# wildminder/ComfyUI-KEEP

Measured on AMD Instinct MI355X. Metric: restored 512x512 face frames/sec, T=20 clip, higher is better.
Workload: dtype f16x3; 1 GPU; 48 independent clips x T=20 x 512x512 per GPU (BASELINE configs[1] clips), KEEP config, synthetic weights seed 0, precision policy x3; clips_per_gpu=48, clip_length=20, parallelism=dp1 over clips, precision_policy=x3

## Files before the change

comfyui-keep_amd/csrc/keep_attn.hip:

```cpp
#include <math.h>
#include <stdlib.h>

#include <type_traits>

#include "keep_common.h"

static constexpr int KEEP_NT_ATTN_O = 0;


struct AttnP {
  const float* q;
  const float* k;
  const float* v;
  const unsigned short* q16;
  const unsigned short* k16;
  const unsigned short* v16;
  float* o;
  long q_bs, q_ts, q_hs, k_bs, k_ts, k_hs, v_bs, v_ts, v_hs, o_bs, o_ts, o_hs;
  int B, H, Lq, Lk, D, Dv;
  float scale;
  int mode, T, seg_len;
  int img_h, img_w, ksplit, shift, kv_rot, n_img;
  int nslices;
  unsigned flags;
  const _Float16* kv_pack;
  const float* q_amax;
  const float* k_amax;
  const float* v_amax;
};

enum AttnForm {
  ATTN_F32,
  ATTN_BF16,
  ATTN_BF16IN,
  ATTN_X3_NQ8,
  ATTN_X3_NQ16,
  ATTN_X3_NQ0,
  ATTN_X3_PACKED,
  ATTN_X3_SMALL,
  ATTN_X3_TWO_PASS,
  ATTN_X3_SFULL,
  ATTN_X3_SFULL2,
};
struct AttnPlan {
  AttnForm form;
  int waves;
  int dvt;
  bool masked;
  size_t lds;
  int64_t scratch;
};
// ... 878 lines not shown
        pl[j] = (_Float16)(s[st * 8 + j] - (float)h);
      }
#pragma unroll
      for (int j = 0; j < DVT; ++j) {
        const _Float16* vrow = Vt + (j * 32 + l31) * VP + (st * 2 + lhi) * 8;
        const af16x8 vh8 = *reinterpret_cast<const af16x8*>(vrow), vl8 = *reinterpret_cast<const af16x8*>(vrow + 32);
        o[j] = __builtin_amdgcn_mfma_f32_32x32x16_f16(pl, vh8, o[j], 0, 0, 0);
        o[j] = __builtin_amdgcn_mfma_f32_32x32x16_f16(ph, vl8, o[j], 0, 0, 0);
        o[j] = __builtin_amdgcn_mfma_f32_32x32x16_f16(ph, vh8, o[j], 0, 0, 0);
      }
    }
    if (PF && kt + 1 < ntiles) {
      __syncthreads();
      if (PACKED) {
        pk_commit();
      } else {
        k_commit();
        v_commit();
      }
    }
  }

  const float inv_l = inv_sv / l_run;
#pragma unroll
  for (int r = 0; r < 16; ++r) {
    const int qrow = (r & 3) + 8 * (r >> 2) + 4 * lhi;
    const float il = __shfl(inv_l, qrow);
    const int t = q0 + wave * 32 + qrow;
    if (t < p.Lq) {
      const long base = q_offset(p, b, t, p.o_bs, p.o_ts) + (long)head * p.o_hs;
#pragma unroll
      for (int j = 0; j < DVT; ++j) {
        const int dv = dv0 + j * 32 + l31;
        if (dv >= p.Dv) continue;
        if (KEEP_NT_ATTN_O)
          __builtin_nontemporal_store(o[j][r] * il, p.o + base + dv);
        else
          p.o[base + dv] = o[j][r] * il;
      }
    }
  }
}

template <int DC, int DVS>
__global__ __launch_bounds__(256) void attn_pack_kv_x3_kernel(AttnP p, _Float16* out) {
  constexpr int QP = 2 * DC + 8, VP = 72, PKK = 32 * QP / 8, PKV = DVS * VP / 8;
// ... 1149 lines not shown
    KEEP_REQUIRE(a.ksplit > 0 && a.img_h % a.ksplit == 0 && a.img_w % a.ksplit == 0, "keep_attention: bad window split");
    const int wh = a.img_h / a.ksplit, ww = a.img_w / a.ksplit;
    KEEP_REQUIRE(a.Lq == wh * ww && a.Lk == wh * ww, "keep_attention: window mode needs Lq == Lk == window size");
    KEEP_REQUIRE(a.n_img > 0 && a.B == a.n_img * a.ksplit * a.ksplit, "keep_attention: B != n_img*ksplit^2");
    KEEP_REQUIRE(a.shift == 0 || a.shift == wh / 2, "keep_attention: shift=%d must be 0 or img_h/ksplit/2 = %d", a.shift, wh / 2);
    KEEP_REQUIRE(a.kv_rot >= 0 && a.kv_rot < a.n_img, "keep_attention: bad kv_rot");
    KEEP_REQUIRE((long)a.img_h * a.img_w <= 65536, "keep_attention: window mode supports maps of at most 65536 tokens");
  }
  KEEP_REQUIRE((!a.q_amax && !a.k_amax && !a.v_amax) || (a.q_amax && a.k_amax && a.v_amax && a.mode == 0 && a.mma == KEEP_MMA_X3),
               "keep_attention: q/k/v_amax come together, with KEEP_MMA_X3 and mode 0 only");
  p.flags = a.flags;
  p.q = (const float*)a.q; p.k = (const float*)a.k; p.v = (const float*)a.v; p.o = a.o;
  p.q16 = (const unsigned short*)a.q; p.k16 = (const unsigned short*)a.k; p.v16 = (const unsigned short*)a.v;
  p.q_bs = a.q_bs; p.q_ts = a.q_ts; p.q_hs = a.q_hs;
  p.k_bs = a.k_bs; p.k_ts = a.k_ts; p.k_hs = a.k_hs;
  p.v_bs = a.v_bs; p.v_ts = a.v_ts; p.v_hs = a.v_hs;
  p.o_bs = a.o_bs; p.o_ts = a.o_ts; p.o_hs = a.o_hs;
  p.B = a.B; p.H = a.H; p.Lq = a.Lq; p.Lk = a.Lk; p.D = a.D; p.Dv = a.Dv;
  p.scale = a.scale; p.mode = a.mode; p.T = a.T; p.seg_len = a.seg_len;
  p.img_h = a.img_h; p.img_w = a.img_w; p.ksplit = a.ksplit; p.shift = a.shift; p.kv_rot = a.kv_rot;
  p.n_img = a.n_img;
  p.q_amax = a.q_amax; p.k_amax = a.k_amax; p.v_amax = a.v_amax;
  p.kv_pack = nullptr;
  const int dvt = a.Dv <= 32 ? 1 : (a.Dv <= 64 ? 2 : 4);
  p.nslices = cdiv(a.Dv, dvt * 32);
  pl = AttnPlan{ATTN_F32, a.Lq <= 32 ? 1 : 4, dvt, false, 0, 0};

  auto rows16 = [](const void* base, int64_t bs, int64_t ts, int64_t hs, int n) {
    return bs % n == 0 && ts % n == 0 && hs % n == 0 && (uintptr_t)base % 16 == 0;
  };
  const int DC = a.D < 128 ? a.D : 128;
  const size_t ntl = (size_t)(a.Lk + 31) / 32;
  const size_t win_tables = ntl * 32 * 4 + ntl * 16 + ntl * 32;

  if (a.in_dtype == KEEP_BF16) {
    const bool ok = a.mma == KEEP_MMA_BF16 && a.D % 16 == 0 && a.Dv % 8 == 0 && rows16(a.q, a.q_bs, a.q_ts, a.q_hs, 8) &&
                    rows16(a.k, a.k_bs, a.k_ts, a.k_hs, 8) && rows16(a.v, a.v_bs, a.v_ts, a.v_hs, 8);
    KEEP_REQUIRE(ok, "keep_attention: bf16 inputs need KEEP_MMA_BF16, D %% 16 == 0, Dv %% 8 == 0 and 16-byte aligned rows");
    const size_t operands = (size_t)((128 + 64) * (DC + 8) + dvt * 32 * 72) * 2;
    const size_t staging = (size_t)4 * 32 * (dvt * 32 + 4) * 4;
    pl.form = ATTN_BF16IN;
    pl.waves = 4;
    pl.masked = a.mode == 2 && a.shift > 0;
    pl.lds = (128 + 3 * 64 + 3 * 64) * sizeof(long) + 3 * 16 * sizeof(unsigned long long) + (operands > staging ? operands : staging);
    return KEEP_OK;
  }
  const bool qk16 = a.D % 16 == 0 && rows16(a.q, a.q_bs, a.q_ts, a.q_hs, 4) && rows16(a.k, a.k_bs, a.k_ts, a.k_hs, 4);
  if (a.mma == KEEP_MMA_BF16) {
    KEEP_REQUIRE(qk16, "keep_attention: KEEP_MMA_BF16 needs D %% 16 == 0 and 16-byte aligned q/k rows");
    pl.form = ATTN_BF16;
    pl.lds = (size_t)((pl.waves * 32 + 32) * (DC + 8) + dvt * 32 * 40) * 2;
    return KEEP_OK;
  }
  if (a.mma != KEEP_MMA_X3 || !qk16 || (a.flags & KEEP_ATTN_NO_X3)) {
    pl.lds = (size_t)((pl.waves * 32 + 32) * (DC + 1) + 32 * dvt * 32) * sizeof(float);
    return KEEP_OK;
  }
// ... 49 lines not shown

template <class F>
static int with_dvt(int dvt, F f) {
  if (dvt == 1) return f(std::integral_constant<int, 1>{});
  if (dvt == 2) return f(std::integral_constant<int, 2>{});
  return f(std::integral_constant<int, 4>{});
}

extern "C" int32_t keep_sizeof_attention_args(void) { return (int32_t)sizeof(keep_attention_args); }

extern "C" int64_t keep_attention_workspace_bytes(const keep_attention_args* a_in) {
  keep_attention_args a;
  AttnP p;
  AttnPlan pl;
  if (attn_args_in(a_in, a) != KEEP_OK || plan_attention(a, INT64_MAX, p, pl) != KEEP_OK) return 0;
  return pl.scratch;
}

extern "C" int32_t keep_attention(const keep_attention_args* a_in, void* stream) {
  keep_attention_args a;
  const int rc_in = attn_args_in(a_in, a);
  if (rc_in != KEEP_OK) return rc_in;
  KEEP_REQUIRE(a.q && a.k && a.v && a.o, "keep_attention: null tensor pointer");
  AttnP p;
  AttnPlan pl;
  const bool ws_ok = a.workspace && (uintptr_t)a.workspace % 16 == 0;
  const int rc = plan_attention(a, ws_ok ? a.workspace_bytes : 0, p, pl);
  if (rc != KEEP_OK) return rc;
  hipStream_t st = (hipStream_t)stream;
  const bool one_wave = pl.waves == 1;
  switch (pl.form) {
    case ATTN_F32:
      return with_dvt(pl.dvt, [&](auto dvt) {
        return one_wave ? launch_attn<1, decltype(dvt)::value>(p, pl, st) : launch_attn<4, decltype(dvt)::value>(p, pl, st);
      });
    case ATTN_BF16:
      return with_dvt(pl.dvt, [&](auto dvt) {
        return one_wave ? launch_attn_bf16<1, decltype(dvt)::value>(p, pl, st) : launch_attn_bf16<4, decltype(dvt)::value>(p, pl, st);
      });
    case ATTN_BF16IN:
      return with_dvt(pl.dvt, [&](auto dvt) { return launch_attn_bf16in<decltype(dvt)::value>(p, pl, st); });
    case ATTN_X3_NQ8:
      return with_dvt(pl.dvt, [&](auto dvt) {
        return one_wave ? launch_attn_x3_t<1, decltype(dvt)::value, 8>(p, pl, st) : launch_attn_x3_t<4, decltype(dvt)::value, 8>(p, pl, st);
      });
    case ATTN_X3_NQ16:
// ... 300 lines not shown
```

comfyui-keep_amd/engine/hiplib.py:

```python
import ctypes as C
import os

import torch

_HERE = os.path.dirname(os.path.abspath(__file__))
LIB_PATH = os.environ.get('KEEP_HIP_LIB') or os.path.join(os.path.dirname(_HERE), 'csrc', 'libkeep_hip.so')
ABI_VERSION = 23

F32, BF16 = 0, 1
MMA_F32, MMA_BF16, MMA_X3, MMA_X1 = 0, 1, 2, 3
PRO_NONE, PRO_SWISH, PRO_RELU = 0, 1, 2
ACT_NONE, ACT_RELU, ACT_LRELU02, ACT_GELU, ACT_SIGMOID, ACT_LRELU01, ACT_SILU = 0, 1, 2, 3, 4, 5, 6
PAD_ZERO, PAD_REFLECT = 0, 1
UPSAMPLE_X2_PHASES = 2
(CONV_NO_COUT4, CONV_NO_C3, CONV_NO_HALO_F32, CONV_NO_HALO_X3, CONV_NO_GATHER_X3, CONV_NO_PLAIN, CONV_NO_FLATK_F32,
 CONV_SMALL_TILES, CONV_X3_EXACT_ACT, CONV_NO_STREAM, CONV_NO_GEMM_LAT, CONV_GEMM_LAT_WAVES, CONV_GEMM_LAT_TILES, CONV_NO_SMALL_PARTIALS) = (1 << i for i in range(14))
CONV_X1_HALO16 = 1 << 15
CONV_X1_GEMM = 1 << 14
ATTN_NO_PACK, ATTN_NO_SFULL2, ATTN_NO_X3, ATTN_NO_SMALL, ATTN_NO_TWO_PASS = 1, 2, 4, 8, 16

_vp, _i32, _i64, _f32, _u32 = C.c_void_p, C.c_int32, C.c_int64, C.c_float, C.c_uint32
STATUS_NONFINITE_LOGITS, STATUS_NONFINITE_TENSOR = 1, 2


class ConvArgs(C.Structure):
    _fields_ = [('struct_size', _u32), ('flags', _u32), ('inp', _vp), ('weight', _vp), ('bias', _vp), ('out', _vp), ('pro_scale', _vp), ('pro_shift', _vp),
                ('residual', _vp), ('aux', _vp), ('workspace', _vp)] + \
               [(n, _i32) for n in ('N', 'H', 'W', 'Cin', 'Cout', 'KH', 'KW', 'stride', 'pad_t', 'pad_l', 'Ho', 'Wo',
                                    'in_ld', 'out_ld', 'res_ld', 'upsample', 'pro_act', 'epi_act')] + \
               [('aux_w', _f32), ('split_k', _i32), ('dtype', _i32), ('mma', _i32), ('weight_bf16', _vp), ('stats_out', _vp), ('stats_P', _i32), ('bk256', _i32), ('out_dtype', _i32),
                ('weight_x3', _vp), ('x3_acc_scale', _f32), ('x3_in_amax', _vp), ('x3_out_amax', _vp), ('x3_out_amax_zeroed', _i32), ('in2', _vp), ('in2_cin1', _i32), ('pad_mode', _i32),
                ('ln_gamma', _vp), ('ln_beta', _vp), ('ln_eps', _f32), ('plan_ref_images', _i32)]


class ConvPlanOut(C.Structure):
    _fields_ = [('path', _i32), ('split_k', _i32), ('workspace_bytes', _i64), ('stats_rows', _i32), ('stats_P', _i32),
                ('wants_bf16_input', _i32), ('out_bf16_ok', _i32), ('out_amax_ok', _i32), ('kernel', C.c_char * 64)]


class AttnArgs(C.Structure):
    _fields_ = [('struct_size', _u32), ('flags', _u32), ('q', _vp), ('k', _vp), ('v', _vp), ('o', _vp)] + \
               [(n, _i64) for n in ('q_bs', 'q_ts', 'q_hs', 'k_bs', 'k_ts', 'k_hs', 'v_bs', 'v_ts', 'v_hs',
                                    'o_bs', 'o_ts', 'o_hs')] + \
               [(n, _i32) for n in ('B', 'H', 'Lq', 'Lk', 'D', 'Dv')] + [('scale', _f32), ('mode', _i32)] + \
               [(n, _i32) for n in ('T', 'seg_len', 'img_h', 'img_w', 'ksplit', 'shift', 'kv_rot', 'n_img', 'mma', 'in_dtype')] + \
               [('q_amax', _vp), ('k_amax', _vp), ('v_amax', _vp), ('workspace', _vp), ('workspace_bytes', _i64)]


_SIGNATURES = {
    'keep_conv2d': [C.POINTER(ConvArgs), _vp],
    'keep_conv2d_plan': [C.POINTER(ConvArgs), C.POINTER(ConvPlanOut)],
    'keep_attention': [C.POINTER(AttnArgs), _vp],
    'keep_chan_stats': [_vp, _vp, _i32, _i32, _i32, _i32, _i32, _vp],
    'keep_norm_finalize': [_vp, _vp, _vp, _vp, _vp, _i32, _i32, _i32, _i32, _i32, _f32, _vp],
    'keep_group_stats': [_vp, _vp, _vp, _vp, _vp, _i32, _i32, _i32, _i32, _f32, _vp],
    'keep_affine_act': [_vp, _vp, _vp, _vp, _i32, _i32, _i32, _i32, _vp],
    'keep_gm_mlp': [_vp, _vp, _vp, _vp, _vp, _i64, _i32, _vp],
    'keep_token_linear': [_vp, _vp, _vp, _vp, _i64, _i32, _i32, _i32, _vp],
    'keep_gm_ffn_x3': [_vp, _vp, _vp, _f32, _vp, _f32, _vp, _vp, _f32, _vp, _i64, _i32, _i32, _i32, _vp],
    'keep_norm_act_bf16': [_vp, _vp, _vp, _vp, _i32, _i32, _i32, _i32, _i32, _vp],
    'keep_gm_join': [_vp, _vp, _vp, _vp, _vp, _vp, _vp, _i32, _i32, _i32, _vp],
    'keep_bilinear_upscale': [_vp, _vp, _i32, _i32, _i32, _i32, _vp],
    'keep_absmax': [_vp, _vp, _i32, _i64, _i32, _i64, _i64, _i32, _vp],
    'keep_layernorm': [_vp, _vp, _vp, _vp, _vp, _vp, _i32, _vp, _i32, _i32, _f32, _vp],
    'keep_geglu': [_vp, _vp, _i32, _i32, _vp],
    'keep_layernorm_amax': [_vp, _vp, _vp, _vp, _vp, _i32, _i32, _f32, _i32, _vp, _i32, _vp],
    'keep_geglu_amax': [_vp, _vp, _i32, _i32, _i32, _vp, _i32, _vp],
    'keep_argmax_gather': [_vp, _vp, _vp, _vp, _vp, _vp, _i32, _i32, _i32, _vp, _vp],
    'keep_nonfinite_flag': [_vp, _i64, _vp, _vp],
# ... 147 lines not shown
```

comfyui-keep_amd/engine/net.py:

```python
import math
import os

import numpy as np
import torch

from . import hiplib as L
from . import ops
from .arch import (CHANNELS, DEFAULT_ARCH, FUSE_ENCODER_BLOCK, FUSE_GENERATOR_BLOCK, GMFLOW, encoder_blocks,
                   generator_blocks)
from .weights import logical_tensors, pack_blob, validate_state_dict, views

_KNOWN_KW = set(DEFAULT_ARCH) | {
    'gumbel_straight_through', 'gumbel_kl_weight', 'vqgan_path', 'fix_modules', 'flownet_path', 'cfa_nlayers',
    'cross_residual', 'mask_ratio'}


FUSED_GM_MLP = os.environ.get('KEEP_NO_FUSED_MLP') is None
FUSED_GM_FFN_X3 = os.environ.get('KEEP_X3_FUSED_FFN', '1') != '0'
GM_S2D_CONV1 = os.environ.get('KEEP_GM_S2D', '1') != '0'
GM_DEDUP_L0 = os.environ.get('KEEP_GM_DEDUP_L0', '1') != '0'
CHECK_X3_RANGE = os.environ.get('KEEP_X3_NO_RANGE_CHECK') is None
GRAPH_MAX_CLIPS = int(os.environ.get('KEEP_AMD_GRAPH_MAX_CLIPS', '2'))
STREAM_OVERLAP_MAX_CLIPS = int(os.environ.get('KEEP_AMD_OVERLAP_MAX_CLIPS', '2'))
CFT_SPLIT = os.environ.get('KEEP_CFT_SPLIT', '1') != '0'
# ... 125 lines not shown
                 and not n.startswith('flownet.')]
        self._dev_blobx1, self._x1_ranges = ops.make_x1_blob(self._dev_blob, self._index, self.w, names)
        x3 = {(a, b): s for a, b, s in self._x3_scales}
        assert all(x3.get((a, b)) == s for a, b, s in self._x1_ranges), 'x1 and x3 twins must share their per-tensor scales'

    def twin_bytes(self, precision=None):
        precision = self.precision if precision is None else precision
        n = int(self._dev_blob.numel()) if self._dev_blob is not None else (0 if self._blob is None else int(self._blob.size))
        return {'bf16': 2 * n, 'x3': 4 * n, 'f16': 4 * n + 2 * n}.get(precision, 0)

    def _activate_precision(self):
        if self.precision == 'bf16':
            if self._dev_blob16 is None:
                self._dev_blob16 = self._dev_blob.to(torch.bfloat16)
            self.o.set_precision(L.MMA_BF16, self._dev_blob, self._dev_blob16)
        elif self.precision in ('x3', 'f16'):
            if self._dev_blobx3 is None:
                self._make_x3()
            self.o.set_precision(L.MMA_X3, self._dev_blob, None, self._dev_blobx3, 1.0, x3_scales=self._x3_scales)
            if FUSED_GM_FFN_X3:
                for n_ in self.w:
                    if n_.startswith('flownet.') and n_.endswith('.mlp.2.weight') and self.w[n_].shape[0] == 128:
                        self.o.ffn_w2_twin(self.w[n_])
            if ops.UP2_PHASES:
                for i, (kind, _, _) in enumerate(generator_blocks(self.cfg)):
                    if kind == 'up':
                        self.o.up2_twin(self.w[f'generator.blocks.{i}.conv.weight'])
            if self.precision == 'f16':
                if self._dev_blobx1 is None:
                    self._make_x1()
                self.o.set_x1_twin(self._dev_blobx1, self._x1_ranges, flags=0, base_kernel=ops.X3_STREAM_KERNEL)
        else:
            self.o.set_precision(L.MMA_F32, self._dev_blob, None)

    def _upload(self, from_blob=None):
        L.load(check_device=True)
        if from_blob is None:
            if self._pinned is None:
                self._pinned = torch.from_numpy(self._blob).pin_memory()
            from_blob = self._pinned
        self._dev_blob = from_blob.to(self.device, non_blocking=False)
        self._dev_blob16 = self._dev_blobx3 = self._dev_blobx1 = None
        self._graphs = {}
        self.w = views(self._dev_blob, self._index)

    def to(self, device):
# ... 282 lines not shown

    def _gm_resblock(self, x, p, stride):
        w = self.w
        c1, st1 = self.o.conv(x, w[f'{p}.conv1.weight'], None, stride=stride, pad=1, stats=True, bounded=True)
        c2, st2 = self.o.conv(c1, w[f'{p}.conv2.weight'], None, pro=self._inorm(c1, st1), pro_act=L.PRO_RELU, stats=True)
        s2, h2 = self._inorm(c2, st2)
        N, H, Wd, C = c2.shape
        out = torch.empty_like(c2)
        if f'{p}.downsample.0.weight' in w:
            d, std = self.o.conv(x, w[f'{p}.downsample.0.weight'].view(C, 1, 1, -1), w[f'{p}.downsample.0.bias'],
                                 stride=stride, pad=0, ksize=1, stats=True, bounded=True)
            sd, hd = self._inorm(d, std)
            L.call('keep_gm_join', d, sd, hd, c2, s2, h2, out, N, H * Wd, C)
        else:
            L.call('keep_gm_join', x, None, None, c2, s2, h2, out, N, H * Wd, C)
        return out

    def _gm_layer(self, src, tgt, p, ffn, h8, w8, shift, kv_rot, n_img):
        w = self.w
        C = src.shape[-1]
        Ltok = h8 * w8
        wqkv = w[f'{p}.qkv.weight']
        o = torch.empty_like(src)
        if tgt is src:
            qkv = self.o.linear(src, wqkv, out_bf16=True, bounded=True, n_img=n_img)
            q, k, v = qkv, ops.offset(qkv, C), ops.offset(qkv, 2 * C)
            sq = skv = (Ltok * 3 * C, 3 * C, 0)
        else:
            q = self.o.linear(src, wqkv[:C], out_bf16=True, bounded=True, n_img=n_img)
            kv = self.o.linear(tgt, wqkv[C:], out_bf16=True, bounded=True, n_img=n_img)
            k, v = kv, ops.offset(kv, C)
            sq, skv = (Ltok * C, C, 0), (Ltok * 2 * C, 2 * C, 0)
        self.o.attention(q, k, v, o, B=n_img * 4, H=1, Lq=Ltok // 4, Lk=Ltok // 4, D=C, Dv=C, scale=1.0 / (C ** 0.5),
                      q_str=sq, k_str=skv, v_str=skv, o_str=(Ltok * C, C, 0), mode=2, img_h=h8, img_w=w8, ksplit=2,
                      shift=shift, kv_rot=kv_rot, n_img=n_img)
        n1 = (w[f'{p}.norm1.weight'], w[f'{p}.norm1.bias'], 1e-5)
        fuse = self.o.ln_fusable(w[f'{p}.merge.weight'], Ltok)
        if not ffn:
            if fuse:
                return self.o.linear(o, w[f'{p}.merge.weight'], bounded=True, n_img=n_img, ln=n1, residual=src)
            m = self.o.linear(o, w[f'{p}.merge.weight'], bounded=True, n_img=n_img)
            return ops.layernorm(m, n1[0], n1[1], res=src)
        if fuse:
            m = self.o.linear(o, w[f'{p}.merge.weight'], bounded=True, n_img=n_img, ln=n1)
        else:
            m = ops.layernorm(self.o.linear(o, w[f'{p}.merge.weight'], bounded=True, n_img=n_img), n1[0], n1[1])
        if (self.o.mma == L.MMA_X3 and C == 128 and FUSED_GM_FFN_X3 and self.o.x3_twin(w[f'{p}.mlp.0.weight']) is not None):
            return self.o.gm_ffn_x3(src, m, w[f'{p}.mlp.0.weight'], w[f'{p}.mlp.2.weight'], w[f'{p}.norm2.weight'], w[f'{p}.norm2.bias'], 1e-5)
        if self.o.mma == L.MMA_BF16 and C == 128 and FUSED_GM_MLP:
            m2 = self.o.gm_mlp(src, m, w[f'{p}.mlp.0.weight'], w[f'{p}.mlp.2.weight'])
        else:
            if self.o.mma == L.MMA_X3:
                hmid = self.o.linear(src, w[f'{p}.mlp.0.weight'], act=L.ACT_GELU, bounded=True, x2=m, n_img=n_img)
            else:
                hmid = self.o.linear(ops.concat2(src, m), w[f'{p}.mlp.0.weight'], act=L.ACT_GELU, bounded=True, n_img=n_img)
            if self.o.ln_fusable(w[f'{p}.mlp.2.weight'], Ltok):
                return self.o.linear(hmid, w[f'{p}.mlp.2.weight'], bounded=True, n_img=n_img, residual=src,
                                     ln=(w[f'{p}.norm2.weight'], w[f'{p}.norm2.bias'], 1e-5))
            m2 = self.o.linear(hmid, w[f'{p}.mlp.2.weight'], bounded=True, n_img=n_img)
        return ops.layernorm(m2, w[f'{p}.norm2.weight'], w[f'{p}.norm2.bias'], res=src)

    def _gm_backbone(self, img_nchw):
        w = self.w
        pfx = 'flownet.model'
        ws2d = w.get(f'{pfx}.backbone.conv1.weight_s2d') if GM_S2D_CONV1 else None
        if ws2d is not None and img_nchw.shape[2] % 2 == 0 and img_nchw.shape[3] % 2 == 0:
# ... 441 lines not shown
```

comfyui-keep_amd/engine/ops.py:

```python
import bisect
import os

import torch

from . import hiplib as L

TOKEN_LINEAR = os.environ.get('KEEP_NO_TOKEN_LINEAR') is None
UP2_PHASES = os.environ.get('KEEP_X3_UP2', '1') != '0'
FUSE_LN = os.environ.get('KEEP_X3_FUSE_LN', '1') != '0'
USE_BK256 = bool(int(os.environ.get('KEEP_BK256', '0')))
HALO_PRENORM_MINPIX = int(os.environ.get('KEEP_HALO_PRENORM_MINPIX', '0'))

DEBUG_SYNC = os.environ.get('KEEP_DEBUG_SYNC') is not None
X3_STREAM_KERNEL = 'conv3x3_halo_x3s_kernel'
_PLAN_CACHE = {}
POLICY_NAMES = {L.MMA_F32: 'fp32', L.MMA_BF16: 'bf16', L.MMA_X3: 'x3'}
PLAN_REF_IMAGES = int(os.environ.get('KEEP_PLAN_REF_IMAGES', '0') or 0)
DEFAULT_CONV_FLAGS = L.CONV_X3_EXACT_ACT if os.environ.get('KEEP_X3_EXACT_ACT') else 0


class Plan:
    __slots__ = ('split_k', 'ws_floats', 'stats_P', 'wants_bf16_input', 'out_bf16_ok', 'out_amax_ok', 'kernel')

    def __init__(self, o):
        self.split_k = o.split_k
        self.ws_floats = o.workspace_bytes // 4
        self.stats_P = o.stats_P
        self.wants_bf16_input = bool(o.wants_bf16_input)
        self.out_bf16_ok = bool(o.out_bf16_ok)
        self.out_amax_ok = bool(o.out_amax_ok)
        self.kernel = o.kernel.decode()
# ... 31 lines not shown
    def __init__(self):
        self.mma = L.MMA_F32
        self.attn_mma = L.MMA_F32
        self.blob32 = None
        self.blob16 = None
        self.blobx3 = None
        self.x3_acc_scale = 1.0
        self._x3_table = None
        self._up2, self._up2_src = {}, (None, None)
        self.profile = None
        self.amax_arena = None
        self.amax_pos = 0
        self.status = None
        self.arena_generation = 0
        self.flags = DEFAULT_CONV_FLAGS
        self.attn_flags = 0
        self.plan_ref_images = PLAN_REF_IMAGES
        self.blobx1 = None
        self._x1_table = None
        self._x1_route = {}
        self.x1_flags = L.CONV_X1_GEMM
        self.x1_base = L.MMA_X3
        self.x1_base_kernel = None
        self.census = None

    def begin_forward(self, device):
        self.ensure_arena(device)
        self._block.zero_()
        self.amax_pos = 0

    def ensure_arena(self, device):
        device = torch.device(device)
        if self.amax_arena is None or self.amax_arena.device != device:
            self._block = torch.empty((1 << 18) + 4, dtype=torch.float32, device=device)
            self.amax_arena = self._block[4:]
            self.status = self._block[:1].view(torch.int32)
            self.arena_generation += 1

    def set_precision(self, mma, blob32=None, blob16=None, blobx3=None, x3_acc_scale=1.0, x3_scales=None):
        if mma not in (L.MMA_F32, L.MMA_BF16, L.MMA_X3):
            raise ValueError(f"set_precision: {mma!r} is no base policy (single fp16 is a base policy plus set_x1_twin)")
        self._x3_table = ([a for a, _, _ in x3_scales], list(x3_scales)) if x3_scales else None
        self.mma = self.attn_mma = mma
        self.set_x1_twin()
        if blobx3 is not None and (blob32 is not self._up2_src[0] or blobx3 is not self._up2_src[1]):
            self._up2, self._up2_src = {}, (blob32, blobx3)
# ... 43 lines not shown

    def bf16_twin(self, w):
        if self.blob16 is None:
            raise RuntimeError("bf16 policy needs the bf16 blob registered (Ops.set_precision)")
        off = self._blob_off(w)
        return self.blob16[off:off + w.numel()]

    def up2_twin(self, w):
        key = (w.data_ptr(), tuple(w.shape))
        tw = self._up2.get(key)
        if tw is None:
            w4 = up2_phase_weights(w)
            sc = x3_scale_for(float(w4.abs().max()))
            tw = self._up2[key] = (split_x3(w4.reshape(-1, w.shape[-1]), sc).view(-1), 1.0 / sc)
        return tw

    def ffn_w2_twin(self, w2):
        key = ('ffn_w2', w2.data_ptr(), tuple(w2.shape))
        tw = self._up2.get(key)
        if tw is None:
            wp = ffn_w2_perm(w2)
            sc = x3_scale_for(float(wp.abs().max()))
            tw = self._up2[key] = (split_x3(wp, sc).view(-1), 1.0 / sc)
        return tw

    def gm_ffn_x3(self, src, msg, w0, w2, gamma, beta, eps):
        C = src.shape[-1]
        M = src.numel() // C
        out = empty((M, C), src)
        w2p, asc2 = self.ffn_w2_twin(w2)
        if self.profile is not None:
            e0, e1 = torch.cuda.Event(enable_timing=True), torch.cuda.Event(enable_timing=True)
            Hd = w0.shape[0]
            self.profile.append(('gm_ffn_x3_kernel', 2.0 * M * (2 * C * Hd + Hd * C), 1, e0, e1,
                                 3 * M * C * 4 + (2 * C * Hd + Hd * C) * 4, (M // 4096 if M % 4096 == 0 else 1, M, 1, 2 * C, C, 1, 1, 0, False)))
            e0.record()
        L.call('keep_gm_ffn_x3', src, msg, self.x3_twin(w0), float(self.x3_scale_of(w0)), w2p, float(asc2), gamma, beta, float(eps), out,
               M, C, w0.shape[0], 1 if (self.flags & L.CONV_X3_EXACT_ACT) else 0)
        if self.profile is not None:
            self.profile[-1][4].record()
        return out.view(src.shape)

    def x3_twin(self, w):
        if self.blobx3 is None or w.shape[-1] % 16:
            return None
        off = self._blob_off(w)
# ... 132 lines not shown
            self.profile.append((pl.kernel, 2.0 * M * Cout * KH * KW * Cin, pl.split_k, e0, e1, alg_bytes,
                                 (N, H, W, Cin, Cout, KH, stride, int(upsample), pro is not None)))
            e0.record()
        if DEBUG_SYNC:
            import sys
            print(f'[keep] {pl.kernel} N={N} H={H} W={W} ld={ld} Cin={Cin} Cout={Cout} k={KH} s={stride} up={int(upsample)} '
                  f'split={pl.split_k} in_off={in_off} pro={pro is not None}/{pro_act} act={act} res={residual is not None} '
                  f'aux={aux is not None} statsP={pl.stats_P if stats else 0}', file=sys.stderr, flush=True)
        if self.census is not None:
            self.census[pl.kernel] = self.census.get(pl.kernel, 0) + 1
        L.conv2d_launch(a)
        if DEBUG_SYNC:
            torch.cuda.synchronize()
            if not bool(torch.isfinite(out.float()).all()):
                import sys
                print(f'[keep] NON-FINITE output of {pl.kernel}; input finite={bool(torch.isfinite(x.float()).all())} '
                      f'absmax={float(x.float().abs().max()):.4g} pro={None if pro is None else [float(t.abs().max()) for t in pro]} '
                      f'res absmax={None if residual is None else float(residual.abs().max())}', file=sys.stderr, flush=True)
        if self.profile is not None:
            self.profile[-1][4].record()
        return (out, st) if stats else out

    def linear(self, x, w, bias=None, *, act=L.ACT_NONE, residual=None, pro=None, pro_act=L.PRO_NONE, cin=None, in_off=0,
               n_img=None, out_bf16=False, bounded=False, x_amax=None, x2=None, ln=None, want_amax=False):
        shp = x.shape
        ld = shp[-1]
        M = x.numel() // ld
        if n_img is None:
            n_img = shp[0] if x.dim() >= 3 else 1
        assert M % n_img == 0, (tuple(shp), n_img)
        if (TOKEN_LINEAR and self.mma == L.MMA_BF16 and ld == 128 and w.shape[0] in (128, 256, 384) and w.shape[-1] == 128
                and M >= 65536 and act == L.ACT_NONE and residual is None and pro is None and pro_act == L.PRO_NONE
                and cin is None and in_off == 0 and x.dtype == torch.float32 and x.is_contiguous()):
            return self.token_linear(x.view(M, ld), w.view(w.shape[0], 128), bias, out_bf16).reshape(*shp[:-1], w.shape[0])
        x4 = x.reshape(n_img, M // n_img, 1, ld)
        x24 = None if x2 is None else x2.reshape(n_img, M // n_img, 1, x2.shape[-1])
        res4 = None if residual is None else residual.reshape(n_img, M // n_img, 1, residual.shape[-1])
        y = self.conv(x4, w, bias, stride=1, pad=0, ksize=1, pro=pro, pro_act=pro_act, act=act, residual=res4, cin=cin,
                      in_off=in_off, out_bf16=out_bf16, bounded=bounded, x_amax=x_amax, x2=x24, ln=ln, stats='amax' if want_amax else False)
        if want_amax:
            y, st = y
            return y.reshape(*shp[:-1], w.shape[0]), (None if st is None else st.amax)
        return y.reshape(*shp[:-1], w.shape[0])

    def ln_fusable(self, w, rows_per_image):
        return (FUSE_LN and self.mma == L.MMA_X3 and w.shape[0] == 128 and w.shape[-1] % 32 == 0 and rows_per_image % 128 == 0
                and self.x3_twin(w) is not None)

    @staticmethod
    def norm_affine(x, gamma, beta, groups, eps, stats=None):
        N, H, W, C = x.shape
        HW = H * W
        scale = empty((N, C), x)
        shift = empty((N, C), x)
        if stats is not None and stats.part is not None:
            L.call('keep_norm_finalize', stats.part, gamma, beta, scale, shift, N, HW, C, groups, stats.P, float(eps))
            return scale, shift
        assert x.dtype == torch.float32, "bf16 activations carry their statistics from the producing conv's epilogue"
        cpg = C // groups
        if ((cpg % 4 == 0 and HW * cpg <= 32768) or HW <= 1024) and C % 4 == 0 and groups >= 2:
            L.call('keep_group_stats', x, gamma, beta, scale, shift, N, HW, C, groups, float(eps))
            return scale, shift
# ... 24 lines not shown
        if self.amax_arena is not None and self.amax_pos + N <= self.amax_arena.numel():
            out = self.amax_arena[self.amax_pos:self.amax_pos + N]
            self.amax_pos += N
            return out, 1
        return torch.empty((N,), dtype=torch.float32, device=like.device), 0

    def layernorm_amax(self, x, gamma, beta, *, n_img, res=None, eps=1e-5):
        C = x.shape[-1]
        M = x.numel() // C
        out = torch.empty_like(x)
        am, zeroed = self._amax_slots(n_img, x)
        L.call('keep_layernorm_amax', x, gamma, beta, res, out, M, C, float(eps), M // n_img, am, zeroed)
        return out, am

    def geglu_amax(self, x, *, n_img):
        F = x.shape[-1] // 2
        M = x.numel() // (2 * F)
        out = empty((*x.shape[:-1], F), x)
        am, zeroed = self._amax_slots(n_img, x)
        L.call('keep_geglu_amax', x, out, n_img, M // n_img, F, am, zeroed)
        return out, am

    def attention(self, q, k, v, o, *, B, H, Lq, Lk, D, Dv, scale, q_str, k_str, v_str, o_str, mode=0, T=0, seg_len=0,
                  img_h=0, img_w=0, ksplit=0, shift=0, kv_rot=0, n_img=0, mma=None, probe=False, amax=None):
        mma = self.attn_mma if mma is None else mma
        in_dtype = L.F32
        if q.dtype == torch.bfloat16:
            assert k.dtype == torch.bfloat16 and v.dtype == torch.bfloat16
            in_dtype, mma = L.BF16, L.MMA_BF16
        elif mma != L.MMA_F32 and (D % 16 or any(s % 4 for s in (*q_str, *k_str))):
            mma = L.MMA_F32
        given = amax
        amax = (None, None, None)
        if given is not None and all(t is not None and t.numel() == B for t in given) and mma == L.MMA_X3 and mode == 0 and in_dtype == L.F32:
            amax = tuple(given)
        elif probe and mma == L.MMA_X3 and mode == 0 and in_dtype == L.F32:
            amax = (absmax(q, B, Lq, H * D, q_str[1], q_str[0], self), absmax(k, B, Lk, H * D, k_str[1], k_str[0], self),
                    absmax(v, B, Lk, H * Dv, v_str[1], v_str[0], self))
        if DEBUG_SYNC:
            import sys
            print(f'[keep] attention mma={mma} in_dtype={in_dtype} B={B} H={H} Lq={Lq} Lk={Lk} D={D} Dv={Dv} mode={mode}',
                  file=sys.stderr, flush=True)
        L.attention(q=q, k=k, v=v, o=o,
                    q_bs=q_str[0], q_ts=q_str[1], q_hs=q_str[2], k_bs=k_str[0], k_ts=k_str[1], k_hs=k_str[2],
                    v_bs=v_str[0], v_ts=v_str[1], v_hs=v_str[2], o_bs=o_str[0], o_ts=o_str[1], o_hs=o_str[2],
                    B=B, H=H, Lq=Lq, Lk=Lk, D=D, Dv=Dv, scale=float(scale), mode=mode, T=T, seg_len=seg_len,
                    img_h=img_h, img_w=img_w, ksplit=ksplit, shift=shift, kv_rot=kv_rot, n_img=n_img, mma=mma,
                    in_dtype=in_dtype, q_amax=amax[0], k_amax=amax[1], v_amax=amax[2], flags=self.attn_flags)
        if DEBUG_SYNC:
            torch.cuda.synchronize()
            if not bool(torch.isfinite(o).all()):
                import sys
                print(f'[keep] NON-FINITE attention output; q/k/v absmax {float(q.float().abs().max()):.4g} '
                      f'{float(k.float().abs().max()):.4g} {float(v.float().abs().max()):.4g}', file=sys.stderr, flush=True)
        return o

    def token_linear(self, x, w, bias=None, out_bf16=False):
        K = x.shape[-1]
        M = x.numel() // K
        N = w.shape[0]
        out = torch.empty((M, N), dtype=torch.bfloat16 if out_bf16 else torch.float32, device=x.device)
        L.call('keep_token_linear', x, self.bf16_twin(w), bias, out, M, K, N, L.BF16 if out_bf16 else L.F32)
        return out

    def gm_mlp(self, a, b, w0, w2):
        C = a.shape[-1]
        M = a.numel() // C
        out = empty((M, C), a)
        L.call('keep_gm_mlp', a, b, self.bf16_twin(w0), self.bf16_twin(w2), out, M, C)
        return out


def absmax(x, N, R, C, ld, img_stride, ops=None):
    out, zeroed = (empty((N,), x), 0) if ops is None else ops._amax_slots(N, x)
    L.call('keep_absmax', x, out, N, R, C, ld, img_stride, zeroed)
    return out


def concat2(a, b, pad_to=1):
# ... 29 lines not shown
def nhwc_to_nchw(x):
    N, H, W, C = x.shape
    out = empty((N, C, H, W), x)
    L.call('keep_nhwc_to_nchw', x, out, N, C, H * W)
    return out


def split_x3(w2d, scale):
    rows, cin = w2d.shape
    ws = w2d.float() * scale
    hi = ws.to(torch.float16)
    lo = (ws - hi.float()).to(torch.float16)
    out = torch.stack((hi.view(rows, cin // 16, 16), lo.view(rows, cin // 16, 16)), dim=2)
    return out.contiguous().view(torch.int16)


FFN_W2_PERM = (0, 1, 2, 3, 8, 9, 10, 11, 4, 5, 6, 7, 12, 13, 14, 15)


def ffn_w2_perm(w2):
    C, Hd = w2.shape
    idx = torch.tensor(FFN_W2_PERM, device=w2.device)
    return w2.float().view(C, Hd // 16, 16).index_select(2, idx).reshape(C, Hd).contiguous()


def up2_phase_weights(w):
    r = torch.zeros(2, 3, 3, dtype=w.dtype, device=w.device)
    r[0, 0, 0] = 1; r[0, 1, 1] = 1; r[0, 1, 2] = 1
    r[1, 1, 0] = 1; r[1, 1, 1] = 1; r[1, 2, 2] = 1
    w4 = torch.einsum('pak,qbl,oklc->pqoabc', r, r, w.float())
    return w4.reshape(4, w.shape[0], 3, 3, w.shape[3]).contiguous()


def make_x3_blob(dev_blob, index, weights, names):
    bx = torch.zeros(2 * dev_blob.numel(), dtype=torch.int16, device=dev_blob.device)
    table = []
    for n in names:
        off, shape = index[n]
        t = weights[n]
        sc = x3_scale_for(float(t.abs().max()))
        bx[2 * off:2 * (off + t.numel())] = split_x3(t.reshape(-1, shape[-1]), sc).view(-1)
        table.append((int(off), int(off + t.numel()), 1.0 / sc))
    table.sort()
    return bx, table


# ... 30 lines not shown
```

include/keep_hip.h:

```cpp
#ifndef KEEP_HIP_H
#define KEEP_HIP_H

#include <stdint.h>

#ifdef __cplusplus
extern "C" {
#endif

#define KEEP_ABI_VERSION 23
#define KEEP_OK 0
#define KEEP_EINVAL (-1)
#define KEEP_EUNSUP (-2)
#define KEEP_EHIP (-3)

#define KEEP_F32 0
#define KEEP_BF16 1

#define KEEP_MMA_F32 0
#define KEEP_MMA_BF16 1
#define KEEP_MMA_X3 2
#define KEEP_MMA_X1 3

#define KEEP_PRO_NONE 0
#define KEEP_PRO_SWISH 1
// ... 8 lines not shown
#define KEEP_ACT_LRELU01 5

#define KEEP_CONV_NO_COUT4 (1u << 0)
#define KEEP_CONV_NO_C3 (1u << 1)
#define KEEP_CONV_NO_HALO_F32 (1u << 2)
#define KEEP_CONV_NO_HALO_X3 (1u << 3)
#define KEEP_CONV_NO_GATHER_X3 (1u << 4)
#define KEEP_CONV_NO_PLAIN (1u << 5)
#define KEEP_CONV_NO_FLATK_F32 (1u << 6)
#define KEEP_CONV_SMALL_TILES (1u << 7)
#define KEEP_CONV_X3_EXACT_ACT (1u << 8)
#define KEEP_CONV_NO_STREAM (1u << 9)
#define KEEP_CONV_NO_GEMM_LAT (1u << 10)
#define KEEP_CONV_GEMM_LAT_WAVES (1u << 11)
#define KEEP_CONV_NO_SMALL_PARTIALS (1u << 13)
#define KEEP_CONV_GEMM_LAT_TILES (1u << 12)
#define KEEP_CONV_X1_GEMM (1u << 14)
#define KEEP_CONV_X1_HALO16 (1u << 15)
#define KEEP_ATTN_NO_PACK (1u << 0)
#define KEEP_ATTN_NO_SFULL2 (1u << 1)
#define KEEP_ATTN_NO_X3 (1u << 2)
#define KEEP_ATTN_NO_TWO_PASS (1u << 4)
#define KEEP_ATTN_NO_SMALL (1u << 3)

#define KEEP_UPSAMPLE_X2_PHASES 2
#define KEEP_PAD_ZERO 0
#define KEEP_PAD_REFLECT 1

int32_t keep_abi_version(void);
const char* keep_last_error(void);
int32_t keep_device_ok(int32_t dev);

typedef struct {
  uint32_t struct_size;
  uint32_t flags;
  const void* in;
  const float* weight;
  const float* bias;
  void* out;
  const float* pro_scale;
  const float* pro_shift;
  const void* residual;
  const void* aux;
  float* workspace;
  int32_t N, H, W, Cin, Cout, KH, KW, stride, pad_t, pad_l, Ho, Wo;
  int32_t in_ld, out_ld, res_ld;
// ... 39 lines not shown
} keep_conv2d_plan_out;
int32_t keep_conv2d_plan(const keep_conv2d_args* a, keep_conv2d_plan_out* out);

typedef struct {
  uint32_t struct_size;
  uint32_t flags;
  const void* q;
  const void* k;
  const void* v;
  float* o;
  int64_t q_bs, q_ts, q_hs, k_bs, k_ts, k_hs, v_bs, v_ts, v_hs, o_bs, o_ts, o_hs;
  int32_t B, H, Lq, Lk, D, Dv;
  float scale;
  int32_t mode;
  int32_t T, seg_len;
  int32_t img_h, img_w, ksplit, shift, kv_rot, n_img;
  int32_t mma;
  int32_t in_dtype;
  const float* q_amax;
  const float* k_amax;
  const float* v_amax;
  void* workspace;
  int64_t workspace_bytes;
} keep_attention_args;
#define KEEP_ATTENTION_ARGS_V12_SIZE 248
int32_t keep_attention(const keep_attention_args* a, void* stream);
int64_t keep_attention_workspace_bytes(const keep_attention_args* a);

int32_t keep_chan_stats(const float* x, float* part, int32_t N, int32_t HW, int32_t C, int32_t ld, int32_t P,
                        void* stream);
int32_t keep_norm_finalize(const float* part, const float* gamma, const float* beta, float* scale, float* shift,
                           int32_t N, int32_t HW, int32_t C, int32_t G, int32_t P, float eps, void* stream);
int32_t keep_group_stats(const float* x, const float* gamma, const float* beta, float* scale, float* shift, int32_t N,
                         int32_t HW, int32_t C, int32_t G, float eps, void* stream);
int32_t keep_affine_act(const float* x, const float* scale, const float* shift, float* out, int32_t N, int32_t HW,
                        int32_t C, int32_t act, void* stream);
int32_t keep_norm_act_bf16(const void* x, const float* scale, const float* shift, void* out, int32_t N, int32_t HW,
                           int32_t C, int32_t act, int32_t in_dtype , void* stream);
int32_t keep_gm_mlp(const float* a, const float* b, const void* w0_bf16, const void* w2_bf16, float* out, int64_t M,
                    int32_t C, void* stream);
int32_t keep_gm_ffn_x3(const float* src, const float* msg, const void* w0_x3, float w0_acc_scale, const void* w2p_x3, float w2_acc_scale,
                       const float* ln_gamma, const float* ln_beta, float ln_eps, float* out, int64_t M, int32_t C, int32_t hidden,
                       int32_t exact_act, void* stream);
int32_t keep_token_linear(const float* x, const void* w_bf16, const float* bias, void* out, int64_t M, int32_t K, int32_t N,
                          int32_t out_dtype, void* stream);
int32_t keep_gm_join(const float* a, const float* sa, const float* ha, const float* b, const float* sb,
// ... 95 lines not shown
```

Baseline: 288.7 frames/s.

## Fold merge projection into V weights and fuse LayerNorm into attention epilogue

Since the merge linear has no bias and attention output is linear in V, the merge weight is folded into the V slice of the qkv projection (Wm·Wv precomputed in double once). The attention packed-x3 kernel then applies LayerNorm plus an optional residual in its epilogue, with a cross-lane shuffle reduction over 128 channels. This removes a separate merge GEMM and a LayerNorm pass over the token map in each transformer layer. It costs extra registers in the epilogue, only works for the packed x3 form with D=Dv=128 and H=1, and changes rounding because the folded weight goes through x3 splitting.

```diff
diff --git a/comfyui-keep_amd/csrc/keep_attn.hip b/comfyui-keep_amd/csrc/keep_attn.hip
--- a/comfyui-keep_amd/csrc/keep_attn.hip
+++ b/comfyui-keep_amd/csrc/keep_attn.hip
@@ -27,6 +27,9 @@
   const float* q_amax;
   const float* k_amax;
   const float* v_amax;
+  const float* ln_gamma;
+  const float* ln_beta;
+  const float* ln_res;
 };
 
 enum AttnForm {
@@ -951,6 +954,45 @@
   }
 
   const float inv_l = inv_sv / l_run;
+  if constexpr (PACKED && DVT == 4 && NQ == 8) {
+    if (p.ln_gamma) {
+      float lng[4], lnb[4];
+#pragma unroll
+      for (int j = 0; j < 4; ++j) {
+        lng[j] = p.ln_gamma[j * 32 + l31];
+        lnb[j] = p.ln_beta[j * 32 + l31];
+      }
+      long base[16];
+      float rr[16][4];
+#pragma unroll
+      for (int r = 0; r < 16; ++r) {
+        const int t = q0 + wave * 32 + (r & 3) + 8 * (r >> 2) + 4 * lhi;
+        base[r] = t < p.Lq ? q_offset(p, b, t, p.o_bs, p.o_ts) + (long)head * p.o_hs : -1;
+#pragma unroll
+        for (int j = 0; j < 4; ++j) rr[r][j] = (p.ln_res && base[r] >= 0) ? p.ln_res[base[r] + j * 32 + l31] : 0.f;
+      }
+#pragma unroll
+      for (int r = 0; r < 16; ++r) {
+        const int qrow = (r & 3) + 8 * (r >> 2) + 4 * lhi;
+        const float il = __shfl(inv_l, qrow);
+        const float e[4] = {o[0][r] * il, o[1][r] * il, o[2][r] * il, o[3][r] * il};
+        float sm = (e[0] + e[1]) + (e[2] + e[3]);
+#pragma unroll
+        for (int x = 1; x < 32; x <<= 1) sm += __shfl_xor(sm, x);
+        const float mean = sm * (1.0f / 128.0f);
+        const float d[4] = {e[0] - mean, e[1] - mean, e[2] - mean, e[3] - mean};
+        float qq = (d[0] * d[0] + d[1] * d[1]) + (d[2] * d[2] + d[3] * d[3]);
+#pragma unroll
+        for (int x = 1; x < 32; x <<= 1) qq += __shfl_xor(qq, x);
+        const float rstd = 1.0f / sqrtf(qq * (1.0f / 128.0f) + 1e-5f);
+        if (base[r] >= 0) {
+#pragma unroll
+          for (int j = 0; j < 4; ++j) p.o[base[r] + j * 32 + l31] = d[j] * rstd * lng[j] + lnb[j] + rr[r][j];
+        }
+      }
+      return;
+    }
+  }
 #pragma unroll
   for (int r = 0; r < 16; ++r) {
     const int qrow = (r & 3) + 8 * (r >> 2) + 4 * lhi;
@@ -2146,6 +2188,10 @@
   p.n_img = a.n_img;
   p.q_amax = a.q_amax; p.k_amax = a.k_amax; p.v_amax = a.v_amax;
   p.kv_pack = nullptr;
+  const bool ln = (a.flags & KEEP_ATTN_LN_EPILOGUE) != 0;
+  p.ln_gamma = ln ? a.ln_gamma : nullptr;
+  p.ln_beta = ln ? a.ln_beta : nullptr;
+  p.ln_res = ln ? a.ln_residual : nullptr;
   const int dvt = a.Dv <= 32 ? 1 : (a.Dv <= 64 ? 2 : 4);
   p.nslices = cdiv(a.Dv, dvt * 32);
   pl = AttnPlan{ATTN_F32, a.Lq <= 32 ? 1 : 4, dvt, false, 0, 0};
@@ -2157,6 +2203,18 @@
   const size_t ntl = (size_t)(a.Lk + 31) / 32;
   const size_t win_tables = ntl * 32 * 4 + ntl * 16 + ntl * 32;
 
+  if (ln) {
+    const int64_t need = (int64_t)a.B * (int64_t)ntl * ((32 * (2 * 128 + 8) + 128 * 72) * 2L);
+    const bool ok = a.mma == KEEP_MMA_X3 && a.in_dtype == KEEP_F32 && rows16(a.q, a.q_bs, a.q_ts, a.q_hs, 4) &&
+                    rows16(a.k, a.k_bs, a.k_ts, a.k_hs, 4) && a.D == 128 && a.Dv == 128 && a.H == 1 && a.Lq >= 256 &&
+                    !(a.flags & (KEEP_ATTN_NO_X3 | KEEP_ATTN_NO_PACK)) && scratch_avail >= need;
+    if (!ok) {
+      keep_set_error("keep_attention: KEEP_ATTN_LN_EPILOGUE needs the packed x3 form (KEEP_MMA_X3, fp32 tensors with 16-byte aligned rows, "
+                     "D = Dv = 128, H = 1, Lq >= 256, a workspace of %lld bytes); got mma=%d D=%d Dv=%d H=%d Lq=%d workspace=%lld",
+                     (long long)need, a.mma, a.D, a.Dv, a.H, a.Lq, (long long)(scratch_avail == INT64_MAX ? -1 : scratch_avail));
+      return KEEP_EUNSUP;
+    }
+  }
   if (a.in_dtype == KEEP_BF16) {
     const bool ok = a.mma == KEEP_MMA_BF16 && a.D % 16 == 0 && a.Dv % 8 == 0 && rows16(a.q, a.q_bs, a.q_ts, a.q_hs, 8) &&
                     rows16(a.k, a.k_bs, a.k_ts, a.k_hs, 8) && rows16(a.v, a.v_bs, a.v_ts, a.v_hs, 8);
@@ -2252,6 +2310,7 @@
   const int rc_in = attn_args_in(a_in, a);
   if (rc_in != KEEP_OK) return rc_in;
   KEEP_REQUIRE(a.q && a.k && a.v && a.o, "keep_attention: null tensor pointer");
+  KEEP_REQUIRE(!(a.flags & KEEP_ATTN_LN_EPILOGUE) || (a.ln_gamma && a.ln_beta), "keep_attention: KEEP_ATTN_LN_EPILOGUE needs ln_gamma and ln_beta");
   AttnP p;
   AttnPlan pl;
   const bool ws_ok = a.workspace && (uintptr_t)a.workspace % 16 == 0;
diff --git a/comfyui-keep_amd/engine/hiplib.py b/comfyui-keep_amd/engine/hiplib.py
--- a/comfyui-keep_amd/engine/hiplib.py
+++ b/comfyui-keep_amd/engine/hiplib.py
@@ -18,6 +18,7 @@
 CONV_X1_HALO16 = 1 << 15
 CONV_X1_GEMM = 1 << 14
 ATTN_NO_PACK, ATTN_NO_SFULL2, ATTN_NO_X3, ATTN_NO_SMALL, ATTN_NO_TWO_PASS = 1, 2, 4, 8, 16
+ATTN_LN_EPILOGUE = 1 << 5
 
 _vp, _i32, _i64, _f32, _u32 = C.c_void_p, C.c_int32, C.c_int64, C.c_float, C.c_uint32
 STATUS_NONFINITE_LOGITS, STATUS_NONFINITE_TENSOR = 1, 2
@@ -44,7 +45,8 @@
                                     'o_bs', 'o_ts', 'o_hs')] + \
                [(n, _i32) for n in ('B', 'H', 'Lq', 'Lk', 'D', 'Dv')] + [('scale', _f32), ('mode', _i32)] + \
                [(n, _i32) for n in ('T', 'seg_len', 'img_h', 'img_w', 'ksplit', 'shift', 'kv_rot', 'n_img', 'mma', 'in_dtype')] + \
-               [('q_amax', _vp), ('k_amax', _vp), ('v_amax', _vp), ('workspace', _vp), ('workspace_bytes', _i64)]
+               [('q_amax', _vp), ('k_amax', _vp), ('v_amax', _vp), ('workspace', _vp), ('workspace_bytes', _i64),
+                ('ln_gamma', _vp), ('ln_beta', _vp), ('ln_residual', _vp)]
 
 
 _SIGNATURES = {
diff --git a/comfyui-keep_amd/engine/net.py b/comfyui-keep_amd/engine/net.py
--- a/comfyui-keep_amd/engine/net.py
+++ b/comfyui-keep_amd/engine/net.py
@@ -171,6 +171,12 @@
                 for n_ in self.w:
                     if n_.startswith('flownet.') and n_.endswith('.mlp.2.weight') and self.w[n_].shape[0] == 128:
                         self.o.ffn_w2_twin(self.w[n_])
+            if ops.FUSE_ATTN_LN:
+                for n_ in self.w:
+                    if n_.startswith('flownet.model.transformer.layers.') and n_.endswith('.qkv.weight'):
+                        p_ = n_[:-len('.qkv.weight')]
+                        if f'{p_}.merge.weight' in self.w and f'{p_}.merge.bias' not in self.w:
+                            self.o.gm_mv_twin(self.w[n_], self.w[f'{p_}.merge.weight'])
             if ops.UP2_PHASES:
                 for i, (kind, _, _) in enumerate(generator_blocks(self.cfg)):
                     if kind == 'up':
@@ -499,26 +505,36 @@
         Ltok = h8 * w8
         wqkv = w[f'{p}.qkv.weight']
         o = torch.empty_like(src)
+        n1 = (w[f'{p}.norm1.weight'], w[f'{p}.norm1.bias'], 1e-5)
+        fold = (self.o.mma == L.MMA_X3 and self.o.blobx3 is not None and f'{p}.merge.bias' not in w
+                and self.o.attn_ln_fusable(Lq=Ltok // 4, D=C, Dv=C, img_h=h8, img_w=w8))
+        x3 = [{}, {}]
+        if fold:
+            wqkv, tx3, asc = self.o.gm_mv_twin(wqkv, w[f'{p}.merge.weight'])
+            x3 = [dict(wx3=tx3[:2 * C * C], x3_acc_scale=asc), dict(wx3=tx3[2 * C * C:], x3_acc_scale=asc)]
         if tgt is src:
-            qkv = self.o.linear(src, wqkv, out_bf16=True, bounded=True, n_img=n_img)
+            qkv = self.o.linear(src, wqkv, out_bf16=True, bounded=True, n_img=n_img, **({} if not fold else dict(wx3=tx3, x3_acc_scale=asc)))
             q, k, v = qkv, ops.offset(qkv, C), ops.offset(qkv, 2 * C)
             sq = skv = (Ltok * 3 * C, 3 * C, 0)
         else:
-            q = self.o.linear(src, wqkv[:C], out_bf16=True, bounded=True, n_img=n_img)
-            kv = self.o.linear(tgt, wqkv[C:], out_bf16=True, bounded=True, n_img=n_img)
+            q = self.o.linear(src, wqkv[:C], out_bf16=True, bounded=True, n_img=n_img, **x3[0])
+            kv = self.o.linear(tgt, wqkv[C:], out_bf16=True, bounded=True, n_img=n_img, **x3[1])
             k, v = kv, ops.offset(kv, C)
             sq, skv = (Ltok * C, C, 0), (Ltok * 2 * C, 2 * C, 0)
         self.o.attention(q, k, v, o, B=n_img * 4, H=1, Lq=Ltok // 4, Lk=Ltok // 4, D=C, Dv=C, scale=1.0 / (C ** 0.5),
                       q_str=sq, k_str=skv, v_str=skv, o_str=(Ltok * C, C, 0), mode=2, img_h=h8, img_w=w8, ksplit=2,
-                      shift=shift, kv_rot=kv_rot, n_img=n_img)
-        n1 = (w[f'{p}.norm1.weight'], w[f'{p}.norm1.bias'], 1e-5)
+                      shift=shift, kv_rot=kv_rot, n_img=n_img, ln=n1[:2] if fold else None, residual=src if (fold and not ffn) else None)
+        if fold and not ffn:
+            return o
         fuse = self.o.ln_fusable(w[f'{p}.merge.weight'], Ltok)
         if not ffn:
             if fuse:
                 return self.o.linear(o, w[f'{p}.merge.weight'], bounded=True, n_img=n_img, ln=n1, residual=src)
             m = self.o.linear(o, w[f'{p}.merge.weight'], bounded=True, n_img=n_img)
             return ops.layernorm(m, n1[0], n1[1], res=src)
-        if fuse:
+        if fold:
+            m = o
+        elif fuse:
             m = self.o.linear(o, w[f'{p}.merge.weight'], bounded=True, n_img=n_img, ln=n1)
         else:
             m = ops.layernorm(self.o.linear(o, w[f'{p}.merge.weight'], bounded=True, n_img=n_img), n1[0], n1[1])
diff --git a/comfyui-keep_amd/engine/ops.py b/comfyui-keep_amd/engine/ops.py
--- a/comfyui-keep_amd/engine/ops.py
+++ b/comfyui-keep_amd/engine/ops.py
@@ -7,6 +7,7 @@
 
 TOKEN_LINEAR = os.environ.get('KEEP_NO_TOKEN_LINEAR') is None
 UP2_PHASES = os.environ.get('KEEP_X3_UP2', '1') != '0'
+FUSE_ATTN_LN = os.environ.get('KEEP_X3_FUSE_ATTN_LN', '1') != '0'
 FUSE_LN = os.environ.get('KEEP_X3_FUSE_LN', '1') != '0'
 USE_BK256 = bool(int(os.environ.get('KEEP_BK256', '0')))
 HALO_PRENORM_MINPIX = int(os.environ.get('KEEP_HALO_PRENORM_MINPIX', '0'))
@@ -84,6 +85,7 @@
         self.x1_flags = L.CONV_X1_GEMM
         self.x1_base = L.MMA_X3
         self.x1_base_kernel = None
+        self._attn_ln = {}
         self.census = None
 
     def begin_forward(self, device):
@@ -173,6 +175,17 @@
             wp = ffn_w2_perm(w2)
             sc = x3_scale_for(float(wp.abs().max()))
             tw = self._up2[key] = (split_x3(wp, sc).view(-1), 1.0 / sc)
+        return tw
+
+    def gm_mv_twin(self, wqkv, wm):
+        key = ('gm_mv', wqkv.data_ptr(), tuple(wqkv.shape))
+        tw = self._up2.get(key)
+        if tw is None:
+            C = wqkv.shape[1]
+            assert tuple(wqkv.shape) == (3 * C, C) and tuple(wm.shape) == (C, C) and C % 16 == 0, (tuple(wqkv.shape), tuple(wm.shape))
+            wmv = fold_merge(wqkv, wm)
+            sc = x3_scale_for(float(wmv.abs().max()))
+            tw = self._up2[key] = (wmv, split_x3(wmv, sc).view(-1), 1.0 / sc)
         return tw
 
     def gm_ffn_x3(self, src, msg, w0, w2, gamma, beta, eps):
@@ -351,7 +364,7 @@
         return (out, st) if stats else out
 
     def linear(self, x, w, bias=None, *, act=L.ACT_NONE, residual=None, pro=None, pro_act=L.PRO_NONE, cin=None, in_off=0,
-               n_img=None, out_bf16=False, bounded=False, x_amax=None, x2=None, ln=None, want_amax=False):
+               n_img=None, out_bf16=False, bounded=False, x_amax=None, x2=None, ln=None, want_amax=False, wx3=None, x3_acc_scale=None):
         shp = x.shape
         ld = shp[-1]
         M = x.numel() // ld
@@ -366,7 +379,8 @@
         x24 = None if x2 is None else x2.reshape(n_img, M // n_img, 1, x2.shape[-1])
         res4 = None if residual is None else residual.reshape(n_img, M // n_img, 1, residual.shape[-1])
         y = self.conv(x4, w, bias, stride=1, pad=0, ksize=1, pro=pro, pro_act=pro_act, act=act, residual=res4, cin=cin,
-                      in_off=in_off, out_bf16=out_bf16, bounded=bounded, x_amax=x_amax, x2=x24, ln=ln, stats='amax' if want_amax else False)
+                      in_off=in_off, out_bf16=out_bf16, bounded=bounded, x_amax=x_amax, x2=x24, ln=ln, stats='amax' if want_amax else False,
+                      wx3=wx3, x3_acc_scale=x3_acc_scale)
         if want_amax:
             y, st = y
             return y.reshape(*shp[:-1], w.shape[0]), (None if st is None else st.amax)
@@ -437,8 +451,9 @@
         return out, am
 
     def attention(self, q, k, v, o, *, B, H, Lq, Lk, D, Dv, scale, q_str, k_str, v_str, o_str, mode=0, T=0, seg_len=0,
-                  img_h=0, img_w=0, ksplit=0, shift=0, kv_rot=0, n_img=0, mma=None, probe=False, amax=None):
+                  img_h=0, img_w=0, ksplit=0, shift=0, kv_rot=0, n_img=0, mma=None, probe=False, amax=None, ln=None, residual=None):
         mma = self.attn_mma if mma is None else mma
+        assert ln is not None or residual is None, 'a residual rides on the LayerNorm epilogue'
         in_dtype = L.F32
         if q.dtype == torch.bfloat16:
             assert k.dtype == torch.bfloat16 and v.dtype == torch.bfloat16
@@ -461,7 +476,9 @@
                     v_bs=v_str[0], v_ts=v_str[1], v_hs=v_str[2], o_bs=o_str[0], o_ts=o_str[1], o_hs=o_str[2],
                     B=B, H=H, Lq=Lq, Lk=Lk, D=D, Dv=Dv, scale=float(scale), mode=mode, T=T, seg_len=seg_len,
                     img_h=img_h, img_w=img_w, ksplit=ksplit, shift=shift, kv_rot=kv_rot, n_img=n_img, mma=mma,
-                    in_dtype=in_dtype, q_amax=amax[0], k_amax=amax[1], v_amax=amax[2], flags=self.attn_flags)
+                    in_dtype=in_dtype, q_amax=amax[0], k_amax=amax[1], v_amax=amax[2],
+                    flags=self.attn_flags | (L.ATTN_LN_EPILOGUE if ln is not None else 0),
+                    ln_gamma=None if ln is None else ln[0], ln_beta=None if ln is None else ln[1], ln_residual=residual)
         if DEBUG_SYNC:
             torch.cuda.synchronize()
             if not bool(torch.isfinite(o).all()):
@@ -470,6 +487,19 @@
                       f'{float(k.float().abs().max()):.4g} {float(v.float().abs().max()):.4g}', file=sys.stderr, flush=True)
         return o
 
+    def attn_ln_fusable(self, *, Lq, D, Dv, img_h, img_w, ksplit=2):
+        if not FUSE_ATTN_LN or self.attn_mma != L.MMA_X3 or D % 16:
+            return False
+        key = (Lq, D, Dv, img_h, img_w, ksplit, self.attn_flags)
+        ok = self._attn_ln.get(key)
+        if ok is None:
+            a = L.AttnArgs(struct_size=L.C.sizeof(L.AttnArgs), flags=self.attn_flags | L.ATTN_LN_EPILOGUE, q_bs=img_h * img_w * D, q_ts=D,
+                           k_bs=img_h * img_w * D, k_ts=D, v_bs=img_h * img_w * Dv, v_ts=Dv, o_bs=img_h * img_w * Dv, o_ts=Dv,
+                           B=ksplit * ksplit, H=1, Lq=Lq, Lk=Lq, D=D, Dv=Dv, scale=1.0, mode=2, img_h=img_h, img_w=img_w, ksplit=ksplit,
+                           n_img=1, mma=L.MMA_X3, in_dtype=L.F32)
+            ok = self._attn_ln[key] = L.attention_workspace_bytes(a) > 0
+        return ok
+
     def token_linear(self, x, w, bias=None, out_bf16=False):
         K = x.shape[-1]
         M = x.numel() // K
@@ -545,6 +575,11 @@
     C, Hd = w2.shape
     idx = torch.tensor(FFN_W2_PERM, device=w2.device)
     return w2.float().view(C, Hd // 16, 16).index_select(2, idx).reshape(C, Hd).contiguous()
+
+
+def fold_merge(wqkv, wm):
+    C = wqkv.shape[1]
+    return torch.cat([wqkv[:2 * C], (wm.double() @ wqkv[2 * C:].double()).float()], dim=0).contiguous()
 
 
 def up2_phase_weights(w):
diff --git a/include/keep_hip.h b/include/keep_hip.h
--- a/include/keep_hip.h
+++ b/include/keep_hip.h
@@ -54,6 +54,7 @@
 #define KEEP_ATTN_NO_X3 (1u << 2)
 #define KEEP_ATTN_NO_TWO_PASS (1u << 4)
 #define KEEP_ATTN_NO_SMALL (1u << 3)
+#define KEEP_ATTN_LN_EPILOGUE (1u << 5)
 
 #define KEEP_UPSAMPLE_X2_PHASES 2
 #define KEEP_PAD_ZERO 0
@@ -139,6 +140,9 @@
   const float* v_amax;
   void* workspace;
   int64_t workspace_bytes;
+  const float* ln_gamma;
+  const float* ln_beta;
+  const float* ln_residual;
 } keep_attention_args;
 #define KEEP_ATTENTION_ARGS_V12_SIZE 248
 int32_t keep_attention(const keep_attention_args* a, void* stream);
```

After: 290.5 frames/s, median of 6. No clear change (+0.6%).
